# anuragranj/cc

Measured on AMD Instinct MI355X. Metric: train images/sec (832x256, 5-frame sample, 6-scale CC step), higher is better.
Workload: dtype f32; 1 GPU; full CC: DispResNet6+PoseNetB6+MaskNet6+Back2Future, all losses; per_gpu_batch=4, global_batch=4, height=256, width=832, scales=6, frames=5, parallelism=dp1, hipgraph=True, trained_nets=all, rccl_ranks=1, dead_occlusion_decoders_elided=False, net_streams=2, pipeline=per_network, grad_chunks=False, deterministic=True

## Files before the change

### cc_amd/csrc/conv_wgrad.hip

```cpp
#include <stdio.h>
#include <stddef.h>
#include <string.h>
#include "cc_common.h"
#include "conv_internal.h"
#include "cc_tools.h"
#include "../../include/ccengine.h"

namespace {

typedef float f32x16 __attribute__((ext_vector_type(16)));

using ccint::BK;
using ccint::BN;
using ccint::MAXGRP;
using ccint::pick_bm;

struct WG {
    const float* a;
    const float* x;
    float* out;
    const float* ga[MAXGRP]; const float* gxp[MAXGRP]; float* gout[MAXGRP];
    int nsplit;
    int B, M, AH, AW; long a_bs;
    int Cin, IH, IW; long x_bs;
    int Rt, St, dy0, dx0, dstep, si;
    long o_sm, o_sc; int o_ri, o_sj;
    int direct, accum;
    int pix_per_split;
};

template <int BM>
__device__ __forceinline__ void wgrad_body(const WG& g, const int bx_, const int by_, const int bz_) {
    const int grp = bz_ / g.nsplit, zsplit = bz_ - grp * g.nsplit;
    const float* __restrict__ a_ = g.ga[grp];
    const float* __restrict__ x_ = g.gxp[grp];
    float* __restrict__ out_ = g.gout[grp];
    constexpr int WM = (BM >= 64) ? BM / 2 : 32;
    constexpr int WN = (BM >= 64) ? 64 : 32;
    constexpr int TM = WM / 32, TN = WN / 32;
    constexpr int AP = BM + 4, BP = BN + 4;
    constexpr int AQ = BM / 16;
    __shared__ float As[2][BK * AP];
    __shared__ float Bs[2][BK * BP];

    const int tid = threadIdx.x, lane = tid & 63;
    const int wid = __builtin_amdgcn_readfirstlane(tid >> 6);
    const int wm = (BM >= 64) ? (wid >> 1) : 0;
    const int wn = (BM >= 64) ? (wid & 1) : wid;
    const int m0 = by_ * BM;
    const int n0 = bx_ * BN;
    const int RS = g.Rt * g.St;
    const int Ntot = g.Cin * RS;
    const int HWa = g.AH * g.AW;
    const long Ptot = (long)g.B * HWa;
    const long pbeg = (long)zsplit * g.pix_per_split;
    long pend = pbeg + g.pix_per_split;
    if (pend > Ptot) pend = Ptot;
    const int x_cs = g.IH * g.IW;

    const int pp = tid & 15, rgp = tid >> 4;
    int xoff[8], tdy[8], tdx[8];
#pragma unroll
    for (int q = 0; q < 8; q++) {
        const int jn = n0 + rgp + 16 * q;
        if (jn < Ntot) {
            const int c = jn / RS, rem = jn - c * RS;
            const int i = rem / g.St, j = rem - i * g.St;
            tdy[q] = g.dy0 + i * g.dstep;
            tdx[q] = g.dx0 + j * g.dstep;
            xoff[q] = c * x_cs + tdy[q] * g.IW + tdx[q];
        } else {
            tdy[q] = -(1 << 28);
            tdx[q] = 0;
            xoff[q] = 0;
        }
    }
    float ra[AQ], rb[8];
    unsigned okA = 0, okB = 0;
    auto load_chunk = [&](long pbase) {
        okA = 0;
        okB = 0;
        const long p = pbase + pp;
        const bool pv = p < pend;
        const long ps = pv ? p : 0;
        const int n = (int)(ps / HWa);
        const int t = (int)(ps - (long)n * HWa);
        const int ty = t / g.AW, tx = t - ty * g.AW;
        const long abase = (long)n * g.a_bs + ty * g.AW + tx;
#pragma unroll
        for (int q = 0; q < AQ; q++) {
            const int m = m0 + rgp + 16 * q;
            const bool ok = pv && (m < g.M);
            ra[q] = a_[ok ? abase + (long)m * HWa : 0];
            okA |= (ok ? 1u : 0u) << q;
        }
        const int iy0 = g.si * ty, ix0 = g.si * tx;
        const long xb = (long)n * g.x_bs + (long)iy0 * g.IW + ix0;
#pragma unroll
        for (int q = 0; q < 8; q++) {
            const int iy = iy0 + tdy[q], ix = ix0 + tdx[q];
            const bool ok = pv && ((unsigned)iy < (unsigned)g.IH) && ((unsigned)ix < (unsigned)g.IW);
            rb[q] = x_[ok ? xb + xoff[q] : 0];
            okB |= (ok ? 1u : 0u) << q;
        }
    };
    auto store_chunk = [&](int buf) {
#pragma unroll
        for (int q = 0; q < AQ; q++) As[buf][pp * AP + rgp + 16 * q] = ((okA >> q) & 1u) ? ra[q] : 0.f;
#pragma unroll
        for (int q = 0; q < 8; q++) Bs[buf][pp * BP + rgp + 16 * q] = ((okB >> q) & 1u) ? rb[q] : 0.f;
    };

    f32x16 acc[TM][TN];
#pragma unroll
    for (int a = 0; a < TM; a++)
#pragma unroll
        for (int b = 0; b < TN; b++)
#pragma unroll
            for (int r = 0; r < 16; r++) acc[a][b][r] = 0.f;

    const int l31 = lane & 31, lk = lane >> 5;
    const long nchunks = (pend > pbeg) ? (pend - pbeg + BK - 1) / BK : 0;
    if (nchunks > 0) {
        load_chunk(pbeg);
        store_chunk(0);
    }
    __syncthreads();
    for (long ch = 0; ch < nchunks; ch++) {
        const int buf = (int)(ch & 1);
        if (ch + 1 < nchunks) load_chunk(pbeg + (ch + 1) * BK);
        {
            float af[BK / 2][TM], bf[BK / 2][TN];
#pragma unroll
            for (int ks = 0; ks < BK / 2; ks++) {
#pragma unroll
                for (int a = 0; a < TM; a++) af[ks][a] = As[buf][(2 * ks + lk) * AP + wm * WM + a * 32 + l31];
#pragma unroll
                for (int b = 0; b < TN; b++) bf[ks][b] = Bs[buf][(2 * ks + lk) * BP + wn * WN + b * 32 + l31];
            }
#pragma unroll
            for (int ks = 0; ks < BK / 2; ks++)
#pragma unroll
                for (int a = 0; a < TM; a++)
#pragma unroll
                    for (int b = 0; b < TN; b++)
                        acc[a][b] = __builtin_amdgcn_mfma_f32_32x32x2f32(af[ks][a], bf[ks][b], acc[a][b], 0, 0, 0);
        }
        if (ch + 1 < nchunks) store_chunk(buf ^ 1);
        __syncthreads();
    }
#pragma unroll
    for (int b = 0; b < TN; b++) {
        const int jn = n0 + wn * WN + b * 32 + l31;
        if (jn >= Ntot) continue;
        long obase;
        if (g.direct) {
            const int c = jn / RS, rem = jn - c * RS;
            const int i = rem / g.St, j = rem - i * g.St;
            obase = (long)c * g.o_sc + i * g.o_ri + j * g.o_sj;
        } else {
            obase = (long)zsplit * g.M * Ntot + jn;
        }
#pragma unroll
        for (int a = 0; a < TM; a++)
#pragma unroll
            for (int r = 0; r < 16; r++) {
                const int m = m0 + wm * WM + a * 32 + (r & 3) + 8 * (r >> 2) + 4 * lk;
                if (m < g.M) {
                    float* o = out_ + obase + (g.direct ? (long)m * g.o_sm : (long)m * Ntot);
                    *o = (g.direct && g.accum) ? (*o + acc[a][b][r]) : acc[a][b][r];
                }
            }
    }
}

template <int BM>
__global__ __launch_bounds__(256) void k_wgrad(WG g) {
    if constexpr (CC_XCD_MASK & 4) {
        const int gx = (int)gridDim.x, gy = (int)gridDim.y;
        const int b = cc_xcd_order((int)blockIdx.x + gx * ((int)blockIdx.y + gy * (int)blockIdx.z), gx * gy * (int)gridDim.z);
        const int r = b / gx;
        wgrad_body<BM>(g, b - r * gx, r % gy, r / gy);
    } else {
        wgrad_body<BM>(g, (int)blockIdx.x, (int)blockIdx.y, (int)blockIdx.z);
    }
}

constexpr int MAXWCLS = 12;
struct WGM { WG c[MAXWCLS]; int n; int bx_end[MAXWCLS]; int gx[MAXWCLS], gy[MAXWCLS]; };
template <int BM>
__global__ __launch_bounds__(256) void k_wgrad_multi(WGM a) {
    int k = 0, first = 0, end = a.bx_end[0];
#pragma unroll
    for (int q = 0; q < MAXWCLS - 1; q++)
        if (q + 1 < a.n && (int)blockIdx.x >= a.bx_end[q]) { k = q + 1; first = a.bx_end[q]; end = a.bx_end[q + 1]; }
#if defined(__HIP_DEVICE_COMPILE__) && !defined(CC_HIPEMU)
    const WG& g = *(reinterpret_cast<const WG*>((const char*)__builtin_amdgcn_kernarg_segment_ptr() + offsetof(WGM, c)) + k);
#else
    const WG& g = a.c[k];
#endif
    const int b = (CC_XCD_MASK & 4) ? cc_xcd_order((int)blockIdx.x - first, end - first) : (int)blockIdx.x - first;
    const int gx = a.gx[k], gy = a.gy[k];
    const int bx = b % gx, r = b / gx;
    wgrad_body<BM>(g, bx, r % gy, r / gy);
}

constexpr int W3_PC = 41;

struct W3 {
    const float* a; const float* x; const float* zeros; float* ws;
    const float* ga[MAXGRP]; const float* gxp[MAXGRP]; float* gws[MAXGRP];
    int B, M, AH, AW; long a_bs;
    int Cin; long x_bs;
    int tiles_x, tiles_y, ntiles, tiles_per_split, nsplit, Cpad, dbg;
};

template <int MT, int CT>
__global__ __launch_bounds__(256, 2) void k_wgrad3x3(W3 g) {
    const float* __restrict__ a_ = g.ga[blockIdx.y];
    const float* __restrict__ x_ = g.gxp[blockIdx.y];
    float* __restrict__ ws_ = g.gws[blockIdx.y];
    constexpr int BM = 32 * MT, BC = 32 * CT;
    constexpr int A_SLOTS = BM * 16;
    constexpr int P_SLOTS = ((BC * W3_PC + 63) / 64) * 64;
    HIP_DYNAMIC_SHARED(float, smem)
    float4* As = reinterpret_cast<float4*>(smem);
    float4* Ps = reinterpret_cast<float4*>(smem) + A_SLOTS;

    const int tid = threadIdx.x, lane = tid & 63;
    const int wid = __builtin_amdgcn_readfirstlane(tid >> 6);
    const int l31 = lane & 31, lk = lane >> 5;
    const int ctiles = g.Cpad / BC;
    const int ctile = blockIdx.x % ctiles, mtile = blockIdx.x / ctiles;
    const int m0 = mtile * BM, c0 = ctile * BC;
    const int HW = g.AH * g.AW;
    const int pt_beg = blockIdx.z * g.tiles_per_split;
    int pt_end = pt_beg + g.tiles_per_split;
    if (pt_end > g.ntiles) pt_end = g.ntiles;

    int g_row[3], g_mt[3], g_ct[3];
    f32x16 acc[3][3];
#pragma unroll
    for (int k = 0; k < 3; k++) {
        const int gi = wid + 4 * k;
        g_row[k] = gi % 3;
        const int tl = gi / 3;
        g_mt[k] = tl % MT;
        g_ct[k] = tl / MT;
#pragma unroll
        for (int j = 0; j < 3; j++)
#pragma unroll
            for (int r = 0; r < 16; r++) acc[k][j][r] = 0.f;
    }

    auto load_tile = [&](int pt) {
        const int tile_x = pt % g.tiles_x;
        const int r2 = pt / g.tiles_x;
        const int tile_y = r2 % g.tiles_y;
        const int n = r2 / g.tiles_y;
        const int ty0 = tile_y * 2, tx0 = tile_x * 32;
        for (int s0 = wid * 64; s0 < A_SLOTS; s0 += 256) {
            const int sl = s0 + lane;
            const int mm = sl >> 4, sc = sl & 15;
            const int pc = sc ^ (mm & 15);
            const int ty = ty0 + (pc >> 3), tx = tx0 + 4 * (pc & 7);
            const int m = m0 + mm;
            const bool ok = (m < g.M) && (ty < g.AH) && (tx < g.AW);
            const float* src = ok ? a_ + (long)n * g.a_bs + (long)m * HW + (long)ty * g.AW + tx : g.zeros;
            __builtin_amdgcn_global_load_lds(CC_GLOBAL_PTR(src), CC_LDS_PTR(As + s0), 16, 0, 0);
        }
        for (int s0 = wid * 64; s0 < P_SLOTS; s0 += 256) {
            const int sl = s0 + lane;
            const int cc = sl / W3_PC, r = sl - cc * W3_PC;
            const int py = r / 10, ch = r - py * 10;
            const int iy = ty0 - 1 + py, ix = tx0 - 4 + 4 * ch;
            const int c = c0 + cc;
            const bool ok = (cc < BC) && (r < 40) && (c < g.Cin) && ((unsigned)iy < (unsigned)g.AH) && ((unsigned)ix < (unsigned)g.AW);
            const float* src = ok ? x_ + (long)n * g.x_bs + (long)c * HW + (long)iy * g.AW + ix : g.zeros;
            __builtin_amdgcn_global_load_lds(CC_GLOBAL_PTR(src), CC_LDS_PTR(Ps + s0), 16, 0, 0);
        }
    };

    for (int pt = pt_beg; pt < pt_end; pt++) {
        if (pt > pt_beg) __syncthreads();
        if (!(g.dbg & 1) || pt == pt_beg) load_tile(pt);
        CC_WAIT_VMCNT0();
        __syncthreads();
        if (g.dbg & 2) continue;
#pragma unroll
        for (int row = 0; row < 2; row++) {
#pragma unroll 2
            for (int pq = 0; pq < 4; pq++) {
#pragma unroll
                for (int k = 0; k < 3; k++) {
                    const int mrow = g_mt[k] * 32 + l31;
                    float4 av = As[mrow * 16 + ((row * 8 + pq + 4 * lk) ^ (mrow & 15))];
                    const float4* Pr = Ps + (g_ct[k] * 32 + l31) * W3_PC + (row + g_row[k]) * 10 + 4 * lk + pq;
                    float4 w0 = Pr[0], w1 = Pr[1], w2 = Pr[2];
                    CC_KEEP4(av); CC_KEEP4(w0); CC_KEEP4(w1); CC_KEEP4(w2);
                    const float a[4] = {av.x, av.y, av.z, av.w};
                    const float w[12] = {w0.x, w0.y, w0.z, w0.w, w1.x, w1.y, w1.z, w1.w, w2.x, w2.y, w2.z, w2.w};
#pragma unroll
                    for (int e = 0; e < 4; e++)
#pragma unroll
                        for (int j = 0; j < 3; j++)
                            acc[k][j] = __builtin_amdgcn_mfma_f32_32x32x2f32(a[e], w[3 + j + e], acc[k][j], 0, 0, 0);
                }
            }
        }
    }
#pragma unroll
    for (int k = 0; k < 3; k++) {
#pragma unroll
        for (int j = 0; j < 3; j++) {
            float* o = ws_ + (((long)blockIdx.z * 9 + (g_row[k] * 3 + j)) * g.M) * g.Cpad + c0 + g_ct[k] * 32 + l31;
#pragma unroll
            for (int r = 0; r < 16; r++) {
                const int m = m0 + g_mt[k] * 32 + (r & 3) + 8 * (r >> 2) + 4 * lk;
                if (m < g.M) o[(long)m * g.Cpad] = acc[k][j][r];
            }
        }
    }
}

__global__ void k_zero64(float* p) { p[threadIdx.x] = 0.f; }

struct WgGeom { int B, M, AH, AW, Cin, IH, IW, R, S, si, pad; };

struct W3Plan { bool ok; int mt, nbuf, tiles_x, tiles_y, ntiles, nsplit, tps, Cp32; size_t smem, ws_floats; };

inline W3Plan plan_w3(int B, int M, int AH, int AW, int Cin, int R, int S, int si, int pad, int IH, int IW, int G = 1) {
    W3Plan p = {};
    p.ok = (R == 3 && S == 3 && si == 1 && pad == 1 && IH == AH && IW == AW && (AW % 4) == 0 && AW >= 16 && Cin >= 32 &&
            M >= cctools::env_int("CC_W3_MINM", 64) &&
            !cctools::env_flag("CC_NO_WGRAD3X3"));
    if (!p.ok) return p;
    p.mt = (M > 64) ? 4 : ((M > 32 && Cin > 32) ? 2 : ((Cin > 64) ? 1 : 2));
    p.nbuf = 1;
    const int BM = 32 * p.mt, BC = 32 * (4 / p.mt);
    p.Cp32 = ((Cin + BC - 1) / BC) * BC;
    p.tiles_x = (AW + 31) / 32;
    p.tiles_y = (AH + 1) / 2;
    p.ntiles = B * p.tiles_x * p.tiles_y;
    const long base = (long)((M + BM - 1) / BM) * (p.Cp32 / BC) * (G > 1 ? G : 1);
    long nsplit = (cctools::env_int("CC_W3_SPLIT", 512) + base - 1) / base;
    const long mt_ = cctools::env_int("CC_W3_MINTILES", 3);
    const long cap = (p.ntiles + mt_ - 1) / mt_;
    if (nsplit > cap) nsplit = cap;
    if (nsplit > p.ntiles) nsplit = p.ntiles;
    if (nsplit < 1) nsplit = 1;
    p.tps = (int)((p.ntiles + nsplit - 1) / nsplit);
    p.nsplit = (p.ntiles + p.tps - 1) / p.tps;
    p.smem = (size_t)(BM * 16 + ((BC * W3_PC + 63) / 64) * 64) * 16;
    p.ws_floats = 64 + (size_t)p.nsplit * 9 * M * p.Cp32;
    return p;
}

struct WinoPadPlan { bool ok; int Wp; ccint::WinoWgradPlan wp; size_t pad_floats; };
inline WinoPadPlan wino_pad_plan(int B, int M, int AH, int AW, int Cin, int G) {
    WinoPadPlan p = {};
    if ((AW % 4) == 0 || AH < 2 || cctools::env_flag("CC_NO_WINO_WGRAD_PAD")) return p;
    if (M < cctools::env_int("CC_WWP_MINM", 96) || Cin < cctools::env_int("CC_WWP_MINC", 96)) return p;
    p.Wp = (AW + 3) & ~3;
    p.wp = ccint::wino_wgrad_plan(B, M, AH, p.Wp, Cin, G, cctools::env_int("CC_WWP_MINQ", 64));
    p.ok = p.wp.ok != 0;
    p.pad_floats = ((size_t)B * (Cin + M) * AH * p.Wp + 3) & ~(size_t)3;
    return p;
}

inline long generic_nsplit(long tiles, long P, bool parked) {
    const long target = parked ? cctools::env_int("CC_WGRAD_PARK_TARGET", 256) : cctools::env_int("CC_WGRAD_SPLIT_TARGET", 512);
    long nsplit = (target + tiles - 1) / tiles;
    const long mr = parked ? cctools::env_int("CC_WGRAD_PARK_MINRANGE", 64) : cctools::env_int("CC_WGRAD_MINRANGE", 32);
    const long maxsplit = (P + mr - 1) / mr;
    if (nsplit > maxsplit) nsplit = maxsplit;
    return nsplit < 1 ? 1 : nsplit;
}

enum WgPath { WG_WINO, WG_WINO_PAD, WG_HEAD, WG_THIN, WG_W3, WG_GENERIC };
struct WgCand {
    WgPath path;
    size_t ws_floats;
    char name[64];
    ccint::WinoWgradPlan wino; int Wp;
    ccint::HeadWgradPlan head;
    W3Plan w3;
};
constexpr int WG_MAXCAND = 5;

static int wgrad_candidates(const WgGeom& g, int G, bool sizing, WgCand* out) {
    int n = 0;
    auto add = [&](WgPath path, size_t ws_floats) -> WgCand& {
        out[n] = WgCand{};
        out[n].path = path;
        out[n].ws_floats = ws_floats;
        return out[n++];
    };
    const int pad = sizing ? 1 : g.pad, IH = sizing ? g.AH : g.IH, IW = sizing ? g.AW : g.IW;
    if (g.R == 3 && g.S == 3 && g.si == 1 && pad == 1 && IH == g.AH && IW == g.AW) {
        const ccint::WinoWgradPlan wp = ccint::wino_wgrad_plan(g.B, g.M, g.AH, g.AW, g.Cin, G);
        if (wp.ok) {
            WgCand& c = add(WG_WINO, wp.ws_floats);
            c.wino = wp;
            snprintf(c.name, sizeof c.name, "k_wino_wgrad");
        }
        const WinoPadPlan pp = wino_pad_plan(g.B, g.M, g.AH, g.AW, g.Cin, G);
        if (pp.ok) {
            WgCand& c = add(WG_WINO_PAD, pp.wp.ws_floats + pp.pad_floats);
            c.wino = pp.wp;
            c.Wp = pp.Wp;
            snprintf(c.name, sizeof c.name, "k_wino_wgrad");
        }
        const ccint::HeadWgradPlan hp = g.M <= 2 ? ccint::head_wgrad_plan(g.B, g.M, g.AH, g.AW, g.Cin) : ccint::HeadWgradPlan{};
        if (hp.ok) {
            WgCand& c = add(WG_HEAD, hp.ws_floats);
            c.head = hp;
            snprintf(c.name, sizeof c.name, "k_wgrad_thinm<%d>", g.M);
        }
    }
    {
        char nm[64] = "";
        if (!sizing) ccint::wgrad_thin_name(g.B, g.M, g.AH, g.AW, g.Cin, g.IH, g.IW, g.R, g.S, g.si, g.pad, nm, sizeof nm);
        const size_t wf = ccint::wgrad_thin_ws_floats(g.B, g.M, g.AH, g.AW, g.Cin, g.R, g.S, g.si);
        if (wf && (sizing || nm[0])) memcpy(add(WG_THIN, wf).name, nm, sizeof nm);
    }
    const W3Plan q = plan_w3(g.B, g.M, g.AH, g.AW, g.Cin, g.R, g.S, g.si, pad, IH, IW, G);
    if (q.ok) {
        WgCand& c = add(WG_W3, q.ws_floats);
        c.w3 = q;
        snprintf(c.name, sizeof c.name, "k_wgrad3x3<%d, %d>", q.mt, 4 / q.mt);
    } else {
        const long Ntot = (long)g.Cin * g.R * g.S;
        const int bm = pick_bm(g.M);
        const long nsplit = generic_nsplit(((Ntot + BN - 1) / BN) * ((g.M + bm - 1) / bm), (long)g.B * g.AH * g.AW, false);
        WgCand& c = add(WG_GENERIC, nsplit <= 1 ? 4 : (size_t)nsplit * g.M * Ntot);
        snprintf(c.name, sizeof c.name, "k_wgrad<%d>", bm);
    }
    return n;
}

struct WgradParked { WG g; int bm; dim3 grid; double gflop; };
struct WgradCollector { WgradParked* p; int cap, n; ccint::WinoWgradParked* wino; };

static void launch_wgrad_parked(const WgradCollector& c, hipStream_t s) {
    for (int bm = 128; bm >= 32; bm /= 2) {
        int i = 0;
        while (i < c.n) {
            WGM m = {};
            long blk = 0;
            double gf = 0;
            for (; i < c.n && m.n < MAXWCLS; i++) {
                if (c.p[i].bm != bm) continue;
                const dim3& gr = c.p[i].grid;
                const long nb = (long)gr.x * gr.y * gr.z;
                if (m.n && blk + nb >= (1l << 31)) break;
                m.c[m.n] = c.p[i].g;
                m.gx[m.n] = (int)gr.x; m.gy[m.n] = (int)gr.y;
                blk += nb;
                m.bx_end[m.n] = (int)blk;
                gf += c.p[i].gflop;
                m.n++;
            }
            if (!m.n) break;
            char nm[64];
            snprintf(nm, sizeof nm, "k_wgrad_multi<%d>%s", bm, "");
            cctiming::Scope tsc(nm, gf, s);
            if (bm == 128) hipLaunchKernelGGL(HIP_KERNEL_NAME(k_wgrad_multi<128>), dim3((unsigned)blk), dim3(256), 0, s, m);
            else if (bm == 64) hipLaunchKernelGGL(HIP_KERNEL_NAME(k_wgrad_multi<64>), dim3((unsigned)blk), dim3(256), 0, s, m);
            else hipLaunchKernelGGL(HIP_KERNEL_NAME(k_wgrad_multi<32>), dim3((unsigned)blk), dim3(256), 0, s, m);
        }
    }
}

struct WgCall {
    int G; const long *a, *x, *gw;
    float* ws; size_t stride_f;
    WgGeom g; long a_bs, x_bs, o_sm, o_sc; int accumulate;
    hipStream_t s; ccint::RedSink* sink; const float* zeros64; WgradCollector* park;
    float* area(int k) const { return ws + k * stride_f; }
};
constexpr int WG_DECLINED = 1;

static int emit_slab_reduce(const WgCall& c, float* const* slabs, int nsplit, int Cp) {
    long rd[MAXGRP][ccint::RD_LONGS];
    for (int k = 0; k < c.G; k++) {
        const long d[ccint::RD_LONGS] = {1, (long)slabs[k], (long)c.gw[k], nsplit, c.accumulate, c.o_sm, c.o_sc, 9, c.g.M, c.g.Cin, Cp};
        memcpy(rd[k], d, sizeof d);
    }
    return ccint::wgrad_reduce_emit(c.sink, &rd[0][0], c.G, c.s);
}

static int emit_tile_reduce(const WgCall& c, long nsplit) {
    const WgGeom& g = c.g;
    long rd[MAXGRP][ccint::RD_LONGS];
    for (int k = 0; k < c.G; k++) {
        const long d[ccint::RD_LONGS] = {0, (long)c.area(k), (long)c.gw[k], nsplit, c.accumulate, c.o_sm, c.o_sc, g.M,
                                         (long)g.Cin * g.R * g.S, g.R * g.S, g.S, g.S, 1};
        memcpy(rd[k], d, sizeof d);
    }
    return ccint::wgrad_reduce_emit(c.sink, &rd[0][0], c.G, c.s);
}

static int run_wino(const WgCall& c, const WgCand& cd) {
    const WgGeom& g = c.g;
    const bool padded = cd.path == WG_WINO_PAD;
    const int W = padded ? cd.Wp : g.AW;
    ccint::WinoWgradParked* wpark = c.park ? c.park->wino : nullptr;
    const bool parks = wpark && wpark->n + c.G <= ccint::WINO_WGRAD_PARK_CAP;
    const ccint::WinoWgradPlan wp = parks ? ccint::wino_wgrad_plan_parked(cd.wino, g.M) : cd.wino;
    const size_t slabs = (cd.wino.ws_floats + 3) & ~(size_t)3;
    const float *ap[MAXGRP], *xp[MAXGRP];
    float* wsp[MAXGRP];
    ccint::PadJob jobs[2 * MAXGRP];
    for (int k = 0; k < c.G; k++) {
        ap[k] = (const float*)c.a[k]; xp[k] = (const float*)c.x[k]; wsp[k] = c.area(k) + 64;
        if (padded) {
            float* xpad = c.area(k) + slabs;
            float* apad = xpad + (size_t)g.B * g.Cin * g.AH * W;
            jobs[2 * k] = ccint::PadJob{xp[k], xpad, c.x_bs, g.Cin * g.AH};
            jobs[2 * k + 1] = ccint::PadJob{ap[k], apad, c.a_bs, g.M * g.AH};
            xp[k] = xpad; ap[k] = apad;
        }
    }
    char nm[128];
    int nl = snprintf(nm, sizeof nm, "%s", cd.name);
    if (cctools::env_flag("CC_TIMING_DETAIL")) {
        nl += snprintf(nm + nl, sizeof nm - nl, " G%d B%d M%d C%d %dx%d", c.G, g.B, g.M, g.Cin, g.AH, g.AW);
        if (padded) nl += snprintf(nm + nl, sizeof nm - nl, "(pad %d)", W);
        snprintf(nm + nl, sizeof nm - nl, " k%d wg%d", wp.nsplit, wp.nmb * wp.ncb * c.G * wp.nsplit);
    }
    bool ok;
    {
        cctiming::Scope tsc(nm, 2e-9 * 16.0 * c.G * g.B * ((g.AH + 1) / 2) * ((W + 1) / 2) * (double)g.M * g.Cin, c.s, !parks);
        if (padded) ccint::pad_rows_launch(jobs, 2 * c.G, g.B, g.AW, W, c.s);
        ok = ccint::wino_wgrad_launch(wp, ap, xp, wsp, c.G, g.B, g.M, g.AH, W, padded ? (long)g.M * g.AH * W : c.a_bs, g.Cin,
                                      padded ? (long)g.Cin * g.AH * W : c.x_bs, c.s, wpark);
    }
    return ok ? emit_slab_reduce(c, wsp, wp.nsplit, wp.Cp) : WG_DECLINED;
}

static int run_head(const WgCall& c, const WgCand& cd) {
    const WgGeom& g = c.g;
    const ccint::HeadWgradPlan& hp = cd.head;
    char nm[128];
    const int nl = snprintf(nm, sizeof nm, "%s", cd.name);
    if (cctools::env_flag("CC_TIMING_DETAIL"))
        snprintf(nm + nl, sizeof nm - nl, " G%d B%d M%d C%d %dx%d r3 s1 k%d", c.G, g.B, g.M, g.Cin, g.AH, g.AW, hp.nblk);
    bool ok = true;
    {
        cctiming::Scope tsc(nm, 2e-9 * c.G * g.B * g.AH * g.AW * (double)g.M * g.Cin * 9, c.s);
        for (int k = 0; k < c.G && ok; k++)
            ok = ccint::head_wgrad_launch(hp, (const float*)c.a[k], (const float*)c.x[k], c.area(k), g.B, g.M, g.AH, g.AW, c.a_bs, g.Cin,
                                          c.x_bs, c.s);
    }
    if (!ok) return WG_DECLINED;
    if (cctools::env_flag("CC_HEAD_TRACE"))
        fprintf(stderr, "head wgrad: G%d B%d M%d C%d %dx%d R%d nblk %d\n", c.G, g.B, g.M, g.Cin, g.AH, g.AW, hp.R, hp.nblk);
    return emit_tile_reduce(c, hp.nblk);
}

static int run_thin(const WgCall& c, const WgCand& cd) {
    const WgGeom& g = c.g;
    char nm[128];
    const int nl = snprintf(nm, sizeof nm, "%s", cd.name);
    if (cctools::env_flag("CC_TIMING_DETAIL"))
        snprintf(nm + nl, sizeof nm - nl, " G%d B%d M%d C%d %dx%d r%d s%d", c.G, g.B, g.M, g.Cin, g.AH, g.AW, g.R, g.si);
    cctiming::Scope tsc(nm, 2e-9 * c.G * g.B * g.AH * g.AW * (double)g.M * g.Cin * g.R * g.S, c.s, !ccint::wgrad_thin_parking());
    bool thin = true;
    for (int k = 0; k < c.G && thin; k++)
        thin = ccint::wgrad_thin_launch((const float*)c.a[k], (const float*)c.x[k], (float*)c.gw[k], c.area(k), g.B, g.M, g.AH, g.AW,
                                        c.a_bs, g.Cin, g.IH, g.IW, c.x_bs, g.R, g.S, g.si, g.pad, c.o_sm, c.o_sc, c.accumulate, c.s,
                                        c.sink);
    return thin ? CC_OK : WG_DECLINED;
}

static int run_w3(const WgCall& c, const WgCand& cd) {
    const WgGeom& g = c.g;
    const W3Plan& q = cd.w3;
    W3 w = {};
    w.zeros = c.zeros64 ? c.zeros64 : c.ws;
    for (int k = 0; k < c.G; k++) { w.ga[k] = (const float*)c.a[k]; w.gxp[k] = (const float*)c.x[k]; w.gws[k] = c.area(k) + 64; }
    w.B = g.B; w.M = g.M; w.AH = g.AH; w.AW = g.AW; w.a_bs = c.a_bs; w.Cin = g.Cin; w.x_bs = c.x_bs;
    w.tiles_x = q.tiles_x; w.tiles_y = q.tiles_y; w.ntiles = q.ntiles; w.tiles_per_split = q.tps; w.nsplit = q.nsplit;
    w.Cpad = q.Cp32;
    if (!c.zeros64) hipLaunchKernelGGL(k_zero64, dim3(1), dim3(64), 0, c.s, c.ws);
    const int BM = 32 * q.mt, BC = 32 * (4 / q.mt);
    dim3 grid((unsigned)(((g.M + BM - 1) / BM) * (q.Cp32 / BC)), (unsigned)c.G, (unsigned)q.nsplit);
    w.dbg = cctools::env_int("CC_W3_DBG", 0);
    {
        char nm[128];
        const int nl = snprintf(nm, sizeof nm, "%s", cd.name);
        if (cctools::env_flag("CC_TIMING_DETAIL"))
            snprintf(nm + nl, sizeof nm - nl, " G%d B%d M%d C%d %dx%d k%d wg%d", c.G, g.B, g.M, g.Cin, g.AH, g.AW, q.nsplit,
                     (int)(grid.x * grid.y * grid.z));
        cctiming::Scope tsc(nm, 2e-9 * c.G * g.B * g.AH * g.AW * (double)g.M * g.Cin * 9, c.s);
        if (q.mt == 4) hipLaunchKernelGGL(HIP_KERNEL_NAME(k_wgrad3x3<4, 1>), grid, dim3(256), q.smem, c.s, w);
        else if (q.mt == 2) hipLaunchKernelGGL(HIP_KERNEL_NAME(k_wgrad3x3<2, 2>), grid, dim3(256), q.smem, c.s, w);
        else hipLaunchKernelGGL(HIP_KERNEL_NAME(k_wgrad3x3<1, 4>), grid, dim3(256), q.smem, c.s, w);
    }
    return emit_slab_reduce(c, w.gws, q.nsplit, q.Cp32);
}

static int run_generic(const WgCall& c, const WgCand& cd) {
    const WgGeom& g = c.g;
    const long Ntot = (long)g.Cin * g.R * g.S;
    const long P = (long)g.B * g.AH * g.AW;
    const int bm = pick_bm(g.M);
    const bool parked = c.park && c.park->n < c.park->cap;
    long nsplit = generic_nsplit(((Ntot + BN - 1) / BN) * ((g.M + bm - 1) / bm) * c.G, P, parked);
    long pps = (P + nsplit - 1) / nsplit;
    pps = ((pps + BK - 1) / BK) * BK;
    nsplit = (P + pps - 1) / pps;
    WG w = {};
    w.B = g.B; w.M = g.M; w.AH = g.AH; w.AW = g.AW; w.a_bs = c.a_bs;
    w.Cin = g.Cin; w.IH = g.IH; w.IW = g.IW; w.x_bs = c.x_bs;
    w.Rt = g.R; w.St = g.S; w.dy0 = -g.pad; w.dx0 = -g.pad; w.dstep = 1; w.si = g.si;
    w.o_sm = c.o_sm; w.o_sc = c.o_sc; w.o_ri = g.S; w.o_sj = 1;
    w.direct = (nsplit == 1);
    w.accum = c.accumulate;
    w.nsplit = (int)nsplit;
    for (int k = 0; k < c.G; k++) {
        w.ga[k] = (const float*)c.a[k]; w.gxp[k] = (const float*)c.x[k];
        w.gout[k] = w.direct ? (float*)c.gw[k] : c.area(k);
    }
    w.pix_per_split = (int)pps;
    dim3 grid((unsigned)((Ntot + BN - 1) / BN), (unsigned)((g.M + bm - 1) / bm), (unsigned)(nsplit * c.G));
    const double gflop = 2e-9 * c.G * g.B * g.AH * g.AW * (double)g.M * g.Cin * g.R * g.S;
    if (parked) {
        c.park->p[c.park->n++] = WgradParked{w, bm, grid, gflop};
    } else {
        char nm[128];
        const int nl = snprintf(nm, sizeof nm, "%s", cd.name);
        if (cctools::env_flag("CC_TIMING_DETAIL"))
            snprintf(nm + nl, sizeof nm - nl, " G%d B%d M%d C%d %dx%d r%d s%d k%ld wg%d", c.G, g.B, g.M, g.Cin, g.AH, g.AW, g.R, g.si,
                     (long)nsplit, (int)(grid.x * grid.y * grid.z));
        cctiming::Scope tsc(nm, gflop, c.s);
        if (bm == 128) hipLaunchKernelGGL(HIP_KERNEL_NAME(k_wgrad<128>), grid, dim3(256), 0, c.s, w);
        else if (bm == 64) hipLaunchKernelGGL(HIP_KERNEL_NAME(k_wgrad<64>), grid, dim3(256), 0, c.s, w);
        else hipLaunchKernelGGL(HIP_KERNEL_NAME(k_wgrad<32>), grid, dim3(256), 0, c.s, w);
    }
    return w.direct ? CC_OK : emit_tile_reduce(c, nsplit);
}

}

extern "C" {

size_t cc_conv2d_wgrad_ws_bytes(int B, int M, int AH, int AW, int Cin, int R, int S, int si) {
    const WgGeom g = {B, M, AH, AW, Cin, 0, 0, R, S, si, 0};
    WgCand c[WG_MAXCAND];
    size_t floats = 0;
    for (int G = 1; G <= MAXGRP; G++) {
        const int n = wgrad_candidates(g, G, true, c);
        for (int i = 0; i < n; i++)
            if (c[i].ws_floats > floats) floats = c[i].ws_floats;
    }
    return (floats * sizeof(float) + 15) & ~(size_t)15;
}

static int wgrad_group_impl(int G, const long* a, const long* x, const long* gw, float* ws, int B, int M, int AH, int AW, long a_bs,
                            int Cin, int IH, int IW, long x_bs, int R, int S, int si, int pad, long o_sm, long o_sc, int accumulate,
                            void* stream, ccint::RedSink* sink, const float* zeros64 = nullptr, WgradCollector* park = nullptr) {
    if (G <= 0 || G > MAXGRP || B <= 0 || M <= 0 || Cin <= 0) return CC_ERR_ARG;
    const WgCall c = {G, a, x, gw, ws, cc_conv2d_wgrad_ws_bytes(B, M, AH, AW, Cin, R, S, si) / sizeof(float),
                      WgGeom{B, M, AH, AW, Cin, IH, IW, R, S, si, pad}, a_bs, x_bs, o_sm, o_sc, accumulate,
                      (hipStream_t)stream, sink, zeros64, park};
    WgCand cand[WG_MAXCAND];
    const int n = wgrad_candidates(c.g, G, false, cand);
    for (int i = 0; i < n; i++) {
        const WgCand& cd = cand[i];
        const int r = cd.path == WG_WINO || cd.path == WG_WINO_PAD ? run_wino(c, cd)
                      : cd.path == WG_HEAD ? run_head(c, cd)
                      : cd.path == WG_THIN ? run_thin(c, cd)
                      : cd.path == WG_W3   ? run_w3(c, cd)
                                           : run_generic(c, cd);
        if (r == WG_DECLINED) continue;
        if (r != CC_OK) return CC_ERR_ARG;
        CC_CHECK_LAUNCH();
        return CC_OK;
    }
    return CC_ERR_ARG;
}

int cc_conv2d_wgrad_group(int G, const long* a, const long* x, const long* gw, float* ws, int B, int M, int AH, int AW, long a_bs,
                          int Cin, int IH, int IW, long x_bs, int R, int S, int si, int pad, long o_sm, long o_sc, int accumulate,
                          void* stream) {
    return wgrad_group_impl(G, a, x, gw, ws, B, M, AH, AW, a_bs, Cin, IH, IW, x_bs, R, S, si, pad, o_sm, o_sc, accumulate, stream,
                            nullptr);
}

int cc_conv2d_wgrad_group_defer(int G, const long* a, const long* x, const long* gw, float* ws, int B, int M, int AH, int AW,
                                long a_bs, int Cin, int IH, int IW, long x_bs, int R, int S, int si, int pad, long o_sm, long o_sc,
                                int accumulate, const float* zeros64_or_null, long* red_host, int red_cap, int* nred_host,
                                void* stream) {
    if (!red_host || !nred_host || red_cap < G) return CC_ERR_ARG;
    ccint::RedSink sink = {red_host, red_cap, 0};
    const int r = wgrad_group_impl(G, a, x, gw, ws, B, M, AH, AW, a_bs, Cin, IH, IW, x_bs, R, S, si, pad, o_sm, o_sc, accumulate,
                                   stream, &sink, zeros64_or_null);
    *nred_host = sink.n;
    return r;
}

int cc_conv2d_wgrad_list(int n, const long* desc_host, const float* zeros64_or_null, long* red_host, int red_cap, int* nred_host,
                         void* stream) {
    if (n <= 0 || !desc_host || !red_host || !nred_host) return CC_ERR_ARG;
    hipStream_t s = (hipStream_t)stream;
    constexpr int CAP = 64;
    static thread_local WgradParked parked[CAP];
    static thread_local ccint::WinoWgradParked wino_parked;
    wino_parked.n = 0;
    WgradCollector col = {parked, CAP, 0, cctools::env_flag("CC_NO_WINO_WGRAD_LIST") ? nullptr : &wino_parked};
    ccint::RedSink sink = {red_host, red_cap, 0};
    struct ThinPark {
        hipStream_t s; bool was;
        explicit ThinPark(hipStream_t st) : s(st), was(ccint::wgrad_thin_park(true)) {}
        ~ThinPark() {
            const double gf = ccint::wgrad_thin_parked_gflop();
            if (gf > 0) {
                cctiming::Scope tsc("k_wgrad_thin_multi", gf, s);
                ccint::wgrad_thin_flush(s);
            }
            ccint::wgrad_thin_park(was);
        }
    } thin_park(s);
    for (int i = 0; i < n; i++) {
        const long* d = desc_host + 32l * i;
        const int G = (int)d[0];
        auto bail = [&](int code) {
            launch_wgrad_parked(col, s);
            if (wino_parked.n > 0) ccint::wino_wgrad_launch_parked(&wino_parked, s);
            *nred_host = sink.n;
            return code;
        };
        if (G <= 0 || G > MAXGRP || sink.n + G > red_cap) return bail(CC_ERR_ARG);
        const int before = col.n;
        const int r = wgrad_group_impl(G, d + 1, d + 5, d + 9, (float*)d[13], (int)d[14], (int)d[15], (int)d[16], (int)d[17], d[18],
                                       (int)d[19], (int)d[20], (int)d[21], d[22], (int)d[23], (int)d[24], (int)d[25], (int)d[26], d[27],
                                       d[28], (int)d[29], stream, &sink, zeros64_or_null, &col);
        if (r != CC_OK) return bail(r);
        if (col.n > before && col.p[before].g.direct) {
            bool dup = false;
            for (int j = 0; j < before && !dup; j++)
                if (col.p[j].g.direct)
                    for (int u = 0; u < MAXGRP && !dup; u++)
                        for (int v = 0; v < MAXGRP; v++)
                            if (col.p[j].g.gout[u] && col.p[j].g.gout[u] == col.p[before].g.gout[v]) { dup = true; break; }
            if (dup) {
                const WgradParked keep = col.p[before];
                col.n = before;
                launch_wgrad_parked(col, s);
                col.p[0] = keep;
                col.n = 1;
            }
        }
    }
    launch_wgrad_parked(col, s);
    if (wino_parked.n > 0) {
        double gf = 0;
        for (int i = 0; i < wino_parked.n; i++) gf += wino_parked.d[i].gflop;
        cctiming::Scope tsc("k_wino_wgrad_multi", gf, s);
        ccint::wino_wgrad_launch_parked(&wino_parked, s);
    }
    *nred_host = sink.n;
    CC_CHECK_LAUNCH();
    return CC_OK;
}

int cc_conv2d_wgrad(const float* a, const float* x, float* gw, float* ws, int B, int M, int AH, int AW, long a_bs, int Cin,
                    int IH, int IW, long x_bs, int R, int S, int si, int pad, long o_sm, long o_sc, int accumulate, void* stream) {
    const long ap = (long)a, xp = (long)x, gp = (long)gw;
    return cc_conv2d_wgrad_group(1, &ap, &xp, &gp, ws, B, M, AH, AW, a_bs, Cin, IH, IW, x_bs, R, S, si, pad, o_sm, o_sc, accumulate,
                                 stream);
}

int cc_conv2d_wgrad_kernel(int B, int M, int AH, int AW, int Cin, int IH, int IW, int R, int S, int si, int pad,
                           void* name_out_host, int cap) {
    WgCand c[WG_MAXCAND];
    wgrad_candidates(WgGeom{B, M, AH, AW, Cin, IH, IW, R, S, si, pad}, 1, false, c);
    snprintf((char*)name_out_host, cap, "%s", c[0].name);
    return CC_OK;
}

}
```

Baseline: 250.4 images/s.

## Vectorize generic wgrad loads with swizzled LDS layout and dense 1x1 fast path

Adds a vectorized main loop for the BM=128 generic weight-gradient kernel. It loads activations as float4 along the pixel dimension, stores them into a k-major, XOR-swizzled shared-memory layout, and reads MFMA fragments back with float4 LDS loads. For 1x1, stride-1, unpadded convolutions the input tile is also read densely with float4. Pixel coordinates advance incrementally instead of being recomputed with divisions each chunk. The goal is fewer global and LDS instructions and fewer bank conflicts, at the cost of more code paths, alignment requirements checked on the host, and higher register pressure.

After: 250.6 images/s, median of 4. Within noise of the previous version (+0.1%).

```diff
diff --git a/cc_amd/csrc/conv_wgrad.hip b/cc_amd/csrc/conv_wgrad.hip
--- a/cc_amd/csrc/conv_wgrad.hip
+++ b/cc_amd/csrc/conv_wgrad.hip
@@ -1,6 +1,7 @@
 #include <stdio.h>
 #include <stddef.h>
 #include <string.h>
+#include <type_traits>
 #include "cc_common.h"
 #include "conv_internal.h"
 #include "cc_tools.h"
@@ -27,7 +28,10 @@
     long o_sm, o_sc; int o_ri, o_sj;
     int direct, accum;
     int pix_per_split;
+    int vec;
 };
+
+__device__ __forceinline__ int wv_swz(int r) { return ((r >> 2) ^ (r & 2)) & 3; }
 
 template <int BM>
 __device__ __forceinline__ void wgrad_body(const WG& g, const int bx_, const int by_, const int bz_) {
@@ -40,8 +44,8 @@
     constexpr int TM = WM / 32, TN = WN / 32;
     constexpr int AP = BM + 4, BP = BN + 4;
     constexpr int AQ = BM / 16;
-    __shared__ float As[2][BK * AP];
-    __shared__ float Bs[2][BK * BP];
+    __shared__ __attribute__((aligned(16))) float As[2][BK * AP];
+    __shared__ __attribute__((aligned(16))) float Bs[2][BK * BP];
 
     const int tid = threadIdx.x, lane = tid & 63;
     const int wid = __builtin_amdgcn_readfirstlane(tid >> 6);
@@ -75,42 +79,6 @@
             xoff[q] = 0;
         }
     }
-    float ra[AQ], rb[8];
-    unsigned okA = 0, okB = 0;
-    auto load_chunk = [&](long pbase) {
-        okA = 0;
-        okB = 0;
-        const long p = pbase + pp;
-        const bool pv = p < pend;
-        const long ps = pv ? p : 0;
-        const int n = (int)(ps / HWa);
-        const int t = (int)(ps - (long)n * HWa);
-        const int ty = t / g.AW, tx = t - ty * g.AW;
-        const long abase = (long)n * g.a_bs + ty * g.AW + tx;
-#pragma unroll
-        for (int q = 0; q < AQ; q++) {
-            const int m = m0 + rgp + 16 * q;
-            const bool ok = pv && (m < g.M);
-            ra[q] = a_[ok ? abase + (long)m * HWa : 0];
-            okA |= (ok ? 1u : 0u) << q;
-        }
-        const int iy0 = g.si * ty, ix0 = g.si * tx;
-        const long xb = (long)n * g.x_bs + (long)iy0 * g.IW + ix0;
-#pragma unroll
-        for (int q = 0; q < 8; q++) {
-            const int iy = iy0 + tdy[q], ix = ix0 + tdx[q];
-            const bool ok = pv && ((unsigned)iy < (unsigned)g.IH) && ((unsigned)ix < (unsigned)g.IW);
-            rb[q] = x_[ok ? xb + xoff[q] : 0];
-            okB |= (ok ? 1u : 0u) << q;
-        }
-    };
-    auto store_chunk = [&](int buf) {
-#pragma unroll
-        for (int q = 0; q < AQ; q++) As[buf][pp * AP + rgp + 16 * q] = ((okA >> q) & 1u) ? ra[q] : 0.f;
-#pragma unroll
-        for (int q = 0; q < 8; q++) Bs[buf][pp * BP + rgp + 16 * q] = ((okB >> q) & 1u) ? rb[q] : 0.f;
-    };
-
     f32x16 acc[TM][TN];
 #pragma unroll
     for (int a = 0; a < TM; a++)
@@ -121,23 +89,126 @@
 
     const int l31 = lane & 31, lk = lane >> 5;
     const long nchunks = (pend > pbeg) ? (pend - pbeg + BK - 1) / BK : 0;
-    if (nchunks > 0) {
-        load_chunk(pbeg);
-        store_chunk(0);
-    }
-    __syncthreads();
-    for (long ch = 0; ch < nchunks; ch++) {
-        const int buf = (int)(ch & 1);
-        if (ch + 1 < nchunks) load_chunk(pbeg + (ch + 1) * BK);
+    auto vec_main = [&](auto dense_c) {
+        float* const vA = &As[0][0];
+        float* const vB = &Bs[0][0];
+        constexpr int AQ4 = (BM + 63) / 64;
+        constexpr bool dense = decltype(dense_c)::value;
+        const int aq = tid & 3, ar = tid >> 2;
+        int at;
+        long aoff, doff = 0;
         {
+            const long p4 = pbeg + 4 * aq;
+            const int n = (int)(p4 / HWa);
+            at = (int)(p4 - (long)n * HWa);
+            aoff = (long)n * g.a_bs + at;
+            if constexpr (dense) doff = (long)n * g.x_bs + at;
+        }
+        aoff += (long)(m0 + ar) * HWa;
+        doff += (long)(n0 + ar) * x_cs;
+        const long a_rs = 64l * HWa, d_rs = 64l * x_cs;
+        unsigned rowsA = 0, rowsD = 0;
+#pragma unroll
+        for (int q = 0; q < AQ4; q++) rowsA |= (((ar + 64 * q < BM) && (m0 + ar + 64 * q < g.M)) ? 1u : 0u) << q;
+#pragma unroll
+        for (int q = 0; q < 2; q++) rowsD |= ((dense && (n0 + ar + 64 * q < Ntot)) ? 1u : 0u) << q;
+        int bn, bty, btx;
+        {
+            const long bp = pbeg + pp;
+            bn = (int)(bp / HWa);
+            const int t = (int)(bp - (long)bn * HWa);
+            bty = t / g.AW;
+            btx = t - bty * g.AW;
+        }
+        const int adv_q = BK / g.AW, adv_x = BK - adv_q * g.AW;
+        const int adv_n = adv_q / g.AH, adv_y = adv_q - adv_n * g.AH;
+        int left = (int)(pend - pbeg);
+
+        float4 ra4[AQ4];
+        float rb[8];
+        unsigned okA = 0, okB = 0;
+        auto load_chunk = [&]() {
+            okA = 0;
+            okB = 0;
+            const bool pv4 = 4 * aq < left;
+#pragma unroll
+            for (int q = 0; q < AQ4; q++) {
+                const bool ok = pv4 && ((rowsA >> q) & 1u);
+                ra4[q] = *reinterpret_cast<const float4*>(a_ + (ok ? aoff + q * a_rs : 0));
+                okA |= (ok ? 1u : 0u) << q;
+            }
+            if constexpr (dense) {
+#pragma unroll
+                for (int q = 0; q < 2; q++) {
+                    const bool ok = pv4 && ((rowsD >> q) & 1u);
+                    const float4 v = *reinterpret_cast<const float4*>(x_ + (ok ? doff + q * d_rs : 0));
+                    rb[4 * q] = v.x; rb[4 * q + 1] = v.y; rb[4 * q + 2] = v.z; rb[4 * q + 3] = v.w;
+                    okB |= (ok ? 1u : 0u) << q;
+                }
+            } else {
+                const bool pv = pp < left;
+                const int iy0 = g.si * bty, ix0 = g.si * btx;
+                const long xb = (long)bn * g.x_bs + (long)iy0 * g.IW + ix0;
+#pragma unroll
+                for (int q = 0; q < 8; q++) {
+                    const int iy = iy0 + tdy[q], ix = ix0 + tdx[q];
+                    const bool ok = pv && ((unsigned)iy < (unsigned)g.IH) && ((unsigned)ix < (unsigned)g.IW);
+                    rb[q] = x_[ok ? xb + xoff[q] : 0];
+                    okB |= (ok ? 1u : 0u) << q;
+                }
+                btx += adv_x; bty += adv_y; bn += adv_n;
+                if (btx >= g.AW) { btx -= g.AW; bty++; }
+                if (bty >= g.AH) { bty -= g.AH; bn++; }
+            }
+            left -= BK;
+            at += BK; aoff += BK; doff += BK;
+            if (at >= HWa) { at -= HWa; aoff += g.a_bs - HWa; doff += g.x_bs - HWa; }
+        };
+        const int wA = ar * 16 + (((aq >> 1) ^ wv_swz(ar)) << 2) + 2 * (aq & 1);
+        const int wB = rgp * 16 + (((((pp & 1) << 1) | (pp >> 3)) ^ wv_swz(rgp)) << 2) + ((pp >> 1) & 3);
+        auto store_chunk = [&](int buf) {
+            float* const sa = vA + buf * (BM * 16);
+            float* const sb = vB + buf * (BN * 16);
+#pragma unroll
+            for (int q = 0; q < AQ4; q++)
+                if (BM >= 64 || ar < BM) {
+                    const bool ok = (okA >> q) & 1u;
+                    *reinterpret_cast<float2*>(sa + wA + 1024 * q) = make_float2(ok ? ra4[q].x : 0.f, ok ? ra4[q].z : 0.f);
+                    *reinterpret_cast<float2*>(sa + (wA ^ 8) + 1024 * q) = make_float2(ok ? ra4[q].y : 0.f, ok ? ra4[q].w : 0.f);
+                }
+            if constexpr (dense) {
+#pragma unroll
+                for (int q = 0; q < 2; q++) {
+                    const bool ok = (okB >> q) & 1u;
+                    *reinterpret_cast<float2*>(sb + wA + 1024 * q) = make_float2(ok ? rb[4 * q] : 0.f, ok ? rb[4 * q + 2] : 0.f);
+                    *reinterpret_cast<float2*>(sb + (wA ^ 8) + 1024 * q) = make_float2(ok ? rb[4 * q + 1] : 0.f, ok ? rb[4 * q + 3] : 0.f);
+                }
+            } else {
+#pragma unroll
+                for (int q = 0; q < 8; q++) sb[wB + 256 * q] = ((okB >> q) & 1u) ? rb[q] : 0.f;
+            }
+        };
+        const int fA = (wm * WM + l31) * 16 + (((2 * lk) ^ wv_swz(l31)) << 2);
+        const int fB = (wn * WN + l31) * 16 + (((2 * lk) ^ wv_swz(l31)) << 2);
+
+        auto mma_chunk = [&](int buf) {
+            const float* const sa = vA + buf * (BM * 16);
+            const float* const sb = vB + buf * (BN * 16);
             float af[BK / 2][TM], bf[BK / 2][TN];
 #pragma unroll
-            for (int ks = 0; ks < BK / 2; ks++) {
-#pragma unroll
-                for (int a = 0; a < TM; a++) af[ks][a] = As[buf][(2 * ks + lk) * AP + wm * WM + a * 32 + l31];
-#pragma unroll
-                for (int b = 0; b < TN; b++) bf[ks][b] = Bs[buf][(2 * ks + lk) * BP + wn * WN + b * 32 + l31];
-            }
+            for (int a = 0; a < TM; a++)
+#pragma unroll
+                for (int h = 0; h < 2; h++) {
+                    const float4 v = *reinterpret_cast<const float4*>(sa + (fA ^ (4 * h)) + 512 * a);
+                    af[4 * h][a] = v.x; af[4 * h + 1][a] = v.y; af[4 * h + 2][a] = v.z; af[4 * h + 3][a] = v.w;
+                }
+#pragma unroll
+            for (int b = 0; b < TN; b++)
+#pragma unroll
+                for (int h = 0; h < 2; h++) {
+                    const float4 v = *reinterpret_cast<const float4*>(sb + (fB ^ (4 * h)) + 512 * b);
+                    bf[4 * h][b] = v.x; bf[4 * h + 1][b] = v.y; bf[4 * h + 2][b] = v.z; bf[4 * h + 3][b] = v.w;
+                }
 #pragma unroll
             for (int ks = 0; ks < BK / 2; ks++)
 #pragma unroll
@@ -145,9 +216,92 @@
 #pragma unroll
                     for (int b = 0; b < TN; b++)
                         acc[a][b] = __builtin_amdgcn_mfma_f32_32x32x2f32(af[ks][a], bf[ks][b], acc[a][b], 0, 0, 0);
-        }
-        if (ch + 1 < nchunks) store_chunk(buf ^ 1);
+        };
+        if (nchunks > 0) {
+            load_chunk();
+            store_chunk(0);
+        }
         __syncthreads();
+        for (long ch = 0; ch + 1 < nchunks; ch++) {
+            const int buf = (int)(ch & 1);
+            load_chunk();
+            mma_chunk(buf);
+            __builtin_amdgcn_sched_barrier(0);
+            store_chunk(buf ^ 1);
+            __syncthreads();
+        }
+        if (nchunks > 0) mma_chunk((int)((nchunks - 1) & 1));
+    };
+    const int mode = BM == 128 ? g.vec : 0;
+    if (mode & 2) {
+        if constexpr (BM == 128) vec_main(std::true_type{});
+    } else if (mode & 1) {
+        if constexpr (BM == 128) vec_main(std::false_type{});
+    } else {
+        float ra[AQ], rb[8];
+        unsigned okA = 0, okB = 0;
+        auto load_chunk = [&](long pbase) {
+            okA = 0;
+            okB = 0;
+            const long p = pbase + pp;
+            const bool pv = p < pend;
+            const long ps = pv ? p : 0;
+            const int n = (int)(ps / HWa);
+            const int t = (int)(ps - (long)n * HWa);
+            const int ty = t / g.AW, tx = t - ty * g.AW;
+            const long abase = (long)n * g.a_bs + ty * g.AW + tx;
+#pragma unroll
+            for (int q = 0; q < AQ; q++) {
+                const int m = m0 + rgp + 16 * q;
+                const bool ok = pv && (m < g.M);
+                ra[q] = a_[ok ? abase + (long)m * HWa : 0];
+                okA |= (ok ? 1u : 0u) << q;
+            }
+            const int iy0 = g.si * ty, ix0 = g.si * tx;
+            const long xb = (long)n * g.x_bs + (long)iy0 * g.IW + ix0;
+#pragma unroll
+            for (int q = 0; q < 8; q++) {
+                const int iy = iy0 + tdy[q], ix = ix0 + tdx[q];
+                const bool ok = pv && ((unsigned)iy < (unsigned)g.IH) && ((unsigned)ix < (unsigned)g.IW);
+                rb[q] = x_[ok ? xb + xoff[q] : 0];
+                okB |= (ok ? 1u : 0u) << q;
+            }
+        };
+        auto store_chunk = [&](int buf) {
+#pragma unroll
+            for (int q = 0; q < AQ; q++) As[buf][pp * AP + rgp + 16 * q] = ((okA >> q) & 1u) ? ra[q] : 0.f;
+#pragma unroll
+            for (int q = 0; q < 8; q++) Bs[buf][pp * BP + rgp + 16 * q] = ((okB >> q) & 1u) ? rb[q] : 0.f;
+        };
+
+        if (nchunks > 0) {
+            load_chunk(pbeg);
+            store_chunk(0);
+        }
+        __syncthreads();
+        for (long ch = 0; ch < nchunks; ch++) {
+            const int buf = (int)(ch & 1);
+            if (ch + 1 < nchunks) load_chunk(pbeg + (ch + 1) * BK);
+            {
+                float af[BK / 2][TM], bf[BK / 2][TN];
+#pragma unroll
+                for (int ks = 0; ks < BK / 2; ks++) {
+#pragma unroll
+                    for (int a = 0; a < TM; a++) af[ks][a] = As[buf][(2 * ks + lk) * AP + wm * WM + a * 32 + l31];
+#pragma unroll
+                    for (int b = 0; b < TN; b++) bf[ks][b] = Bs[buf][(2 * ks + lk) * BP + wn * WN + b * 32 + l31];
+                }
+#pragma unroll
+                for (int ks = 0; ks < BK / 2; ks++)
+#pragma unroll
+                    for (int a = 0; a < TM; a++)
+#pragma unroll
+                        for (int b = 0; b < TN; b++)
+                            acc[a][b] = __builtin_amdgcn_mfma_f32_32x32x2f32(af[ks][a], bf[ks][b], acc[a][b], 0, 0, 0);
+            }
+            if (ch + 1 < nchunks) store_chunk(buf ^ 1);
+            __syncthreads();
+        }
     }
 #pragma unroll
     for (int b = 0; b < TN; b++) {
@@ -368,6 +522,19 @@
     return p;
 }
 
+inline int generic_vec_mode(const WgGeom& g, int bm, long a_bs, long x_bs, const long* a, const long* x, int G) {
+    if (bm < 128 || cctools::env_flag("CC_WGRAD_SCALAR")) return 0;
+    const long HWa = (long)g.AH * g.AW;
+    if ((HWa % 4) != 0 || HWa < BK || (a_bs % 4) != 0) return 0;
+    bool dense = g.R == 1 && g.S == 1 && g.si == 1 && g.pad == 0 && g.IH == g.AH && g.IW == g.AW && (x_bs % 4) == 0 &&
+                 !cctools::env_flag("CC_WGRAD_SCALAR_GATHER");
+    for (int k = 0; k < G; k++) {
+        if (a[k] & 15) return 0;
+        if (x[k] & 15) dense = false;
+    }
+    return dense ? 3 : 1;
+}
+
 inline long generic_nsplit(long tiles, long P, bool parked) {
     const long target = parked ? cctools::env_int("CC_WGRAD_PARK_TARGET", 256) : cctools::env_int("CC_WGRAD_SPLIT_TARGET", 512);
     long nsplit = (target + tiles - 1) / tiles;
@@ -624,16 +791,21 @@
         w.gout[k] = w.direct ? (float*)c.gw[k] : c.area(k);
     }
     w.pix_per_split = (int)pps;
+    w.vec = generic_vec_mode(g, bm, c.a_bs, c.x_bs, c.a, c.x, c.G);
     dim3 grid((unsigned)((Ntot + BN - 1) / BN), (unsigned)((g.M + bm - 1) / bm), (unsigned)(nsplit * c.G));
     const double gflop = 2e-9 * c.G * g.B * g.AH * g.AW * (double)g.M * g.Cin * g.R * g.S;
+    if (cctools::env_flag("CC_WGRAD_TRACE"))
+        fprintf(stderr, "generic wgrad: G%d B%d M%d C%d %dx%d in %dx%d r%d s%d bm%d k%ld wg%d %s vec%d gflop %.4f\n", c.G, g.B, g.M, g.Cin,
+                g.AH, g.AW, g.IH, g.IW, g.R, g.si, bm, (long)nsplit, (int)(grid.x * grid.y * grid.z), parked ? "parked" : "alone", w.vec,
+                gflop);
     if (parked) {
         c.park->p[c.park->n++] = WgradParked{w, bm, grid, gflop};
     } else {
         char nm[128];
         const int nl = snprintf(nm, sizeof nm, "%s", cd.name);
         if (cctools::env_flag("CC_TIMING_DETAIL"))
-            snprintf(nm + nl, sizeof nm - nl, " G%d B%d M%d C%d %dx%d r%d s%d k%ld wg%d", c.G, g.B, g.M, g.Cin, g.AH, g.AW, g.R, g.si,
-                     (long)nsplit, (int)(grid.x * grid.y * grid.z));
+            snprintf(nm + nl, sizeof nm - nl, " G%d B%d M%d C%d %dx%d r%d s%d k%ld wg%d v%d", c.G, g.B, g.M, g.Cin, g.AH, g.AW, g.R, g.si,
+                     (long)nsplit, (int)(grid.x * grid.y * grid.z), w.vec);
         cctiming::Scope tsc(nm, gflop, c.s);
         if (bm == 128) hipLaunchKernelGGL(HIP_KERNEL_NAME(k_wgrad<128>), grid, dim3(256), 0, c.s, w);
         else if (bm == 64) hipLaunchKernelGGL(HIP_KERNEL_NAME(k_wgrad<64>), grid, dim3(256), 0, c.s, w);
```
